# nomadkaraoke/python-audio-separator

Hardware: AMD Instinct MI355X
Metric: audio-sec separated / wall-sec (RTF), UVR-MDX-NET 44.1kHz stereo, 1/2/4/8 GPU (higher is better)
Workload: dtype f32 (I/O and accumulators; matrix products on the 16-bit pipe from block-scaled two-part fp16 operands, 22-bit products -- see arithmetic; fp32-exact setting timed in arithmetic_ab)

## Files before the change

python-audio-separator_amd/csrc/asx.hip:

```cpp
#include <hip/hip_runtime.h>

#include <algorithm>
#include <atomic>
#include <cmath>
#include <cstdarg>
#include <cstdio>
#include <cstdlib>
#include <cstring>
#include <functional>
#include <map>
#include <string>
#include <mutex>
#include <vector>

#include "../../include/asx.h"
#include "knobs.h"
#include "resample_plan.h"
#include "flac_dec_plan.h"

static void grant_lds(const void *kernel, int bytes) {
  static std::mutex mu;
  static std::map<const void *, int> granted;
  std::lock_guard<std::mutex> lock(mu);
  int &g = granted[kernel];
// ... 29 lines not shown
#include "kernels_pcm_encode.h"
#include "kernels_flac_dec.h"

using namespace asx;

#include "engine_core.h"
#include "engine_mdx.h"

static int opt_nonneg(int32_t v) { return v < 0 ? 0 : (int)v; }
static int opt_onoff(int32_t v) { return v > 0 ? 1 : 0; }

static const struct EngineOption {
  const char *key;
  int asx_engine::*field;
  int EngineKnobs::*knob;
  int (*norm)(int32_t);
  const char *refusal = nullptr;
  int shipped = 0;
} kOptions[] = {
    {"winograd", &asx_engine::winograd, &EngineKnobs::winograd, opt_nonneg,
     "asx_set_option: winograd = %d names a superseded kernel generation that only an experimental build carries "
     "(python build.py --experimental); this library has 0 (direct kernel) and 3 (the default)", 3},
    {"winograd_stationary", &asx_engine::winos, &EngineKnobs::winos, opt_nonneg,
     "asx_set_option: the weight-stationary Winograd kernel (measured slower) is in experimental builds only (python build.py --experimental)"},
    {"winograd_bf16x6", &asx_engine::wino6, &EngineKnobs::wino6, opt_nonneg},
    {"gemm_bf16x6", &asx_engine::gemm_bf16x6, &EngineKnobs::gemm_bf16x6, opt_onoff},
    {"gemm_f16x3", &asx_engine::gemm_f16x3, &EngineKnobs::gemm_f16x3, opt_onoff},
    {"conv_direct_f16x3", &asx_engine::conv3h, &EngineKnobs::conv3h, opt_nonneg},
    {"conv_fuse_input", &asx_engine::conv_fuse_input, &EngineKnobs::conv_fuse_input, opt_onoff},
    {"tdf_fuse_output", &asx_engine::tdf_fuse_output, &EngineKnobs::tdf_fuse_output, opt_onoff},
    {"conv3h_partial_scratch", &asx_engine::conv3h_ps, &EngineKnobs::conv3h_ps, opt_onoff},
    {"conv3h_walk", &asx_engine::conv3h_walk, &EngineKnobs::conv3h_walk, opt_onoff},
    {"conv3h_tiled", &asx_engine::conv3h_tiled, &EngineKnobs::conv3h_tiled, opt_onoff},
    {"conv_down_bf16x6", &asx_engine::down6, &EngineKnobs::down6, opt_onoff},
    {"conv_up_bf16x6", &asx_engine::up6, &EngineKnobs::up6, opt_onoff},
    {"gemm_pair_images", &asx_engine::pair_images, &EngineKnobs::pair_images, opt_onoff,
     "asx_set_option: gemm_pair_images = 1 needs an experimental build (python build.py --experimental): the pair-image reader measured no "
     "faster in the nets and is not in the default library"},
};

static const EngineOption *find_option(const char *fn, const char *key) {
  for (const EngineOption &o : kOptions)
    if (!strcmp(key, o.key)) return &o;
  set_err("%s: unknown option '%s'", fn, key);
  return nullptr;
}

extern "C" {

int asx_abi_version(void) { return ASX_ABI_VERSION; }
const char *asx_last_error(void) { return g_err; }

int asx_device_count(void) {
  int n = 0;
  if (hipGetDeviceCount(&n) != hipSuccess) return 0;
  return n;
}

int asx_engine_create(int device, const asx_mdx_config *cfg, asx_engine **out) {
  REQUIRE(cfg && out, "asx_engine_create: null argument");
  REQUIRE(cfg->n_fft >= 8 && cfg->n_fft % 2 == 0, "n_fft must be even and >= 8 (got %d)", cfg->n_fft);
  REQUIRE(cfg->hop_length > 0 && cfg->segment_size >= 2, "bad hop_length/segment_size");
  REQUIRE(cfg->dim_f > 0 && cfg->dim_f <= cfg->n_fft / 2 + 1, "dim_f %d out of range for n_fft %d", cfg->dim_f,
          cfg->n_fft);
  REQUIRE(cfg->overlap >= 0.0 && cfg->overlap < 1.0, "overlap must be in [0,1)");
  REQUIRE(cfg->win_length >= 0 && cfg->win_length <= cfg->n_fft, "win_length %d out of range for n_fft %d", cfg->win_length, cfg->n_fft);
// ... 2600 lines not shown

int asx_vr_separate(asx_engine *e, const float *wave_host, int64_t n_samples, const asx_vr_params *params, float *primary_host,
                    float *secondary_host) {
  REQUIRE(e && wave_host && params && n_samples > 0, "asx_vr_separate: bad argument");
  READY(e->vr, "asx_vr_separate");
  HIPCHK(hipSetDevice(e->device));
  int T;
  int64_t n_out;
  CHK(vr_plan(*e->vr, n_samples, &T, &n_out));
  DevBuf dw, dp, ds;
  BufGuard g{{&dw, &dp, &ds}};
  CHK(to_dev(dw, wave_host, (size_t)2 * n_samples));
  if (primary_host) CHK(dp.ensure((size_t)2 * n_out * 4));
  if (secondary_host) CHK(ds.ensure((size_t)2 * n_out * 4));
  CHK(vr_separate_dev(e, dw.f(), n_samples, params, primary_host ? dp.f() : nullptr, secondary_host ? ds.f() : nullptr, nullptr));
  if (primary_host) CHK(to_host(primary_host, dp, (size_t)2 * n_out));
  if (secondary_host) CHK(to_host(secondary_host, ds, (size_t)2 * n_out));
  return ASX_OK;
}

int asx_counter(const asx_engine *e, const char *name, int64_t *out) {
  REQUIRE(e && name && out, "asx_counter: null argument");
  const std::string nm(name);
  if (nm == "tdf3_launches") *out = (int64_t)g_tdf3_launches.load();
  else if (nm == "tdf3h_launches") *out = (int64_t)g_tdf3h_launches.load();
  else if (nm == "attn6_launches") *out = (int64_t)g_attn6_launches.load();
  else if (nm == "attn6h_launches") *out = (int64_t)g_attn6h_launches.load();
  else if (nm == "tdf3_gather_launches") *out = (int64_t)g_tdf3_gather_launches.load();
  else if (nm == "wino6_launches") *out = (int64_t)g_wino6_launches.load();
  else if (nm == "wino6h_launches") *out = (int64_t)g_wino6h_launches.load();
  else if (nm == "conv3h_launches") *out = (int64_t)g_conv3h_launches.load();
  else if (nm == "conv3h_fin_launches") *out = (int64_t)g_conv3h_fin_launches.load();
  else if (nm == "conv3h_tiled_launches") *out = (int64_t)g_conv3h_tiled_launches.load();
  else if (nm == "tdf_fused_output_launches") *out = (int64_t)g_tdf_fused_output_launches.load();
  else if (nm == "tdf3_pair_image_launches") *out = (int64_t)g_tdf3ps_launches.load();
  else if (nm == "down6_launches") *out = (int64_t)g_down6_launches.load();
  else if (nm == "up6_launches") *out = (int64_t)g_up6_launches.load();
  else if (nm == "hd_rounds") *out = (int64_t)g_hd_rounds.load();
  else if (nm == "vr_net_passes") *out = (int64_t)g_vr_net_passes.load();
  else if (nm == "v3_net_passes") *out = (int64_t)g_v3_net_passes.load();
  else if (nm == "rof_net_passes") *out = (int64_t)g_rof_net_passes.load();
  else if (nm == "flac_block_cycles") *out = (int64_t)e->flac_block_cycles;
  else if (nm == "flac_crc16_cycles") *out = (int64_t)e->flac_crc16_cycles;
  else {
    set_err("asx_counter: unknown counter '%s'", name);
    return ASX_ERR_INVALID;
  }
  return ASX_OK;
}

int asx_debug_trace(uint64_t *host, int64_t n_u64) {
  REQUIRE(host && n_u64 > 0 && n_u64 <= 4096 * 8, "asx_debug_trace: bad argument");
  HIPCHK(hipDeviceSynchronize());
  HIPCHK(hipMemcpyFromSymbol(host, HIP_SYMBOL(asx_dbg_trace), (size_t)n_u64 * 8));
  return ASX_OK;
}

int asx_debug_fetch(asx_engine *e, const char *name, float *host, int64_t numel) {
  REQUIRE(e && name && host && numel > 0, "asx_debug_fetch: bad argument");
  HIPCHK(hipSetDevice(e->device));
  const float *src = nullptr;
  const std::string nm(name);
  if (e->vr && e->vr->ws_batch > 0) {
    auto &b = e->vr->b;
    if (nm == "vr.hc") src = b.hc;
    else if (nm == "vr.y2") src = b.y2;
// ... 249 lines not shown
```

python-audio-separator_amd/csrc/conv3h_walk_plan.h:

```cpp
#pragma once
#include <algorithm>
#include <cstdint>
#include <vector>

struct Conv3hUnit {
  int32_t b, band, t0, tiles;
};

struct Conv3hWalkPlan {
  int bw = 32, tps = 0;
  int ngroups = 8;
  std::vector<std::vector<Conv3hUnit>> units;
  int steps(int g) const {
    int n = 0;
    for (const Conv3hUnit &u : units[(size_t)g]) n += u.tiles + 1;
    return n;
  }
  int longest() const {
    int n = 0;
    for (int g = 0; g < ngroups; ++g) n = std::max(n, steps(g));
    return n;
  }
  int max_units() const {
    size_t n = 0;
    for (const auto &l : units) n = std::max(n, l.size());
    return (int)n;
  }
};

static inline int conv3h_walk_bw0(int B, int tilesT, int tilesF) {
  int bw = 32;
  double best = 1e30;
  for (int cand : {32, 16, 8}) {
    if ((tilesT * cand) % 32 != 0) continue;
    const int tps = tilesT * cand / 32;
    const int bands = (tilesF + cand - 1) / cand, items = B * bands;
    const double cost = (double)(bands * cand) / tilesF * (tps + 1.0) / tps * (double)((items + 7) / 8) / (items / 8.0);
    if (cost < best - 1e-9) {
      best = cost;
      bw = cand;
    }
  }
  return best > 1e29 ? 32 : bw;
}

static inline Conv3hWalkPlan conv3h_walk_arith(int B, int tilesT, int tilesF, int bw) {
  Conv3hWalkPlan p;
  p.bw = (tilesT * bw) % 32 == 0 ? bw : 32;
  p.tps = tilesT * p.bw / 32;
  const int segs = 32 / p.bw, nbands = (tilesF + p.bw - 1) / p.bw, items = B * nbands;
  p.ngroups = 8 * segs;
  p.units.assign((size_t)p.ngroups, {});
  for (int x = 0; x < 8; ++x)
    for (int seg = 0; seg < segs; ++seg)
      for (int item = x; item < items; item += 8)
        p.units[(size_t)(x * segs + seg)].push_back({item / nbands, item % nbands, seg * p.tps, p.tps});
  return p;
}
static inline Conv3hWalkPlan conv3h_walk_plan0(int B, int tilesT, int tilesF) { return conv3h_walk_arith(B, tilesT, tilesF, conv3h_walk_bw0(B, tilesT, tilesF)); }

static inline Conv3hWalkPlan conv3h_walk_balanced(int B, int tilesT, int tilesF, int gran, int bw) {
  Conv3hWalkPlan p;
  p.bw = bw;
  p.tps = 0;
  p.ngroups = 256 / bw;
  p.units.assign((size_t)p.ngroups, {});
  const int G = p.ngroups, nbands = (tilesF + bw - 1) / bw, items = B * nbands;
  const int rounds = items / G, left = items - rounds * G;
  for (int r = 0; r < rounds; ++r)
    for (int g = 0; g < G; ++g) {
      const int item = r * G + g;
      p.units[(size_t)g].push_back({item / nbands, item % nbands, 0, tilesT});
    }
  if (left > 0) {
    const int64_t tT = ((int64_t)(tilesT + gran - 1) / gran) * gran, total = (int64_t)left * tT;
    int64_t share = (total + G - 1) / G;
    share = (share + gran - 1) / gran * gran;
    for (int g = 0; g < G; ++g) {
      int64_t lo = (int64_t)g * share;
      const int64_t hi = std::min(total, lo + share);
      while (lo < hi) {
        const int64_t i = lo / tT, t0 = lo - i * tT, t1 = std::min<int64_t>(tT, t0 + (hi - lo));
        const int item = rounds * G + (int)i;
        if (t0 < tilesT) p.units[(size_t)g].push_back({item / nbands, item % nbands, (int)t0, (int)std::min<int64_t>(t1, tilesT) - (int)t0});
        lo += t1 - t0;
      }
    }
  }
  return p;
}

static inline Conv3hWalkPlan conv3h_walk_plan(int B, int tilesT, int tilesF, int gran, int mode) {
  Conv3hWalkPlan best = conv3h_walk_plan0(B, tilesT, tilesF);
  if (mode == 0) return best;
  if (gran < 1) gran = 1;
  int nbest = best.tps % gran == 0 || best.tps == tilesT ? best.longest() : INT32_MAX;
  for (int bw : {32, 16, 8}) {
    Conv3hWalkPlan c = conv3h_walk_balanced(B, tilesT, tilesF, gran, bw);
    const int n = c.longest();
    if (n < nbest) {
      nbest = n;
      best = std::move(c);
    }
  }
  return best;
}

static inline int conv3h_walk_table(const Conv3hWalkPlan &p, std::vector<int32_t> &tab) {
  const int stride = p.max_units() + 2;
  tab.assign((size_t)p.ngroups * stride * 4, 0);
  for (int g = 0; g < p.ngroups; ++g) {
    int32_t *row = &tab[(size_t)g * stride * 4];
    const auto &l = p.units[(size_t)g];
    row[0] = p.steps(g);
    row[1] = (int32_t)l.size();
    for (size_t u = 0; u <= l.size(); ++u) {
      const Conv3hUnit un = u < l.size() ? l[u] : Conv3hUnit{0, 0, 0, 1 << 30};
      int32_t *e = row + 4 * (1 + u);
      e[0] = un.b;
      e[1] = un.band;
      e[2] = un.t0;
      e[3] = un.tiles;
    }
  }
  return stride;
// ... 2 lines not shown
```

python-audio-separator_amd/csrc/engine_core.h:

```cpp
#pragma once

static thread_local char g_err[512] = "";
static void set_err(const char *fmt, ...) {
  va_list ap;
  va_start(ap, fmt);
  vsnprintf(g_err, sizeof(g_err), fmt, ap);
  va_end(ap);
}
#define HIPCHK(x)                                                                       \
  do {                                                                                  \
    hipError_t e_ = (x);                                                                \
    if (e_ != hipSuccess) {                                                             \
      set_err("%s:%d %s -> %s", __FILE__, __LINE__, #x, hipGetErrorString(e_));         \
      return ASX_ERR_HIP;                                                               \
    }                                                                                   \
  } while (0)
#define CHK(x)                    \
  do {                            \
    int r_ = (x);                 \
    if (r_ != ASX_OK) return r_;  \
  } while (0)
#define REQUIRE(cond, ...)        \
  do {                            \
    if (!(cond)) {                \
// ... 80 lines not shown
  DevBuf wd6;
  int wd6_cg = 0, wd6_nst = 0, wd6_nrep = 3;
  DevBuf wup6;
  int wup6_cg = 0, wup6_nst = 0;
};

struct TdfLayer {
  int n = 0, k = 0, c = 0;
  bool has_bias = false;
  DevBuf w, bias, scale, shift;
  DevBuf gn_w, gn_b;
};

struct Block {
  std::vector<ConvLayer> tfc;
  TdfLayer tdf0, tdf1;
  int c = 0, t = 0, f = 0;
};

struct ProfRec {
  int cls;
  int nprod;
  hipEvent_t a, b;
  double flops, bytes;
};

struct RsTable {
  ResamplePlan plan;
  DevBuf tab;
};

struct Conv3hWalkTab {
  int B, tilesT, tilesF, mode;
  int bw, stride;
  DevBuf tab;
};

struct V3Net;
struct RofNet;
struct HtNet;
struct HdNet;
struct VrNet;
struct EnsCtx;

struct W3Entry {
  const float *w;
  int N, K, cin;
  int kind;
  void *img;
};

struct DivKey {
  int64_t N = -1;
  int n_chunks = 0;
  int64_t C = 0, step = 0, L = 0;
  int trim = 0, win = 0;
  int hann_tab = 0;
  bool operator==(const DivKey &o) const {
    return N == o.N && n_chunks == o.n_chunks && C == o.C && step == o.step && L == o.L && trim == o.trim && win == o.win &&
           hann_tab == o.hann_tab;
  }
};

struct asx_engine {
  int device = 0;
  V3Net *v3 = nullptr;
// ... 25 lines not shown
  std::vector<ConvLayer> ds, us;
  int ws_batch = 0;
  DevBuf spec_in, spec_out, R[3], H, HE, frames, chunk_out, d_starts, d_nact, d_peak, d_demixed;
  DevBuf pool_wave, pool_nsong, pool_songs, pool_div, pool_peak;
  DevBuf c3h_ps;
  std::vector<Conv3hWalkTab *> c3h_walks;
  DevBuf gn_part;
  DevBuf d_div;
  DivKey div_key;
  DevBuf sinc_tab;
  DevBuf sinc_jobs;
  DevBuf flac_cycles;
  long long flac_block_cycles = 0, flac_crc16_cycles = 0;
  DevBuf flac_frames, flac_off;
  DevBuf flacdec_list, flacdec_slots, flacdec_accept;
  std::vector<flacdec::Accept> flacdec_accept_host;
  int64_t flacdec_n_samples = -1, flacdec_n_frames = 0;
  int32_t flacdec_channels = 0, flacdec_bps = 0, flacdec_max_bs = 0;
  size_t flacdec_slot_off = 0;
  std::vector<RsTable *> rs_tabs;
  std::mutex rs_mu;
  hipEvent_t div_ev = nullptr;
  hipStream_t div_stream = nullptr;
  std::vector<DevBuf> skip;
  int winograd = 3;
  int winos = 0;
  int gemm_bf16x6 = 1;
  int gemm_f16x3 = 1;
  int wino6 = 144;
  int conv3h = 144;
  int conv3h_ps = 1;
  int conv3h_walk = 1;
  int conv3h_tiled = 1;
  int conv_fuse_input = 1;
  int tdf_fuse_output = 1;
  int down6 = 1;
  int up6 = 1;
  int pair_images = 0;
  std::vector<W3Entry> w3;
  std::mutex w3_mu;
  bool prof = false;
  int prof_nprod = 0;
  std::vector<ProfRec> recs;
};

static int pick_batch(const asx_engine *e) { return e->cfg.max_batch > 0 ? e->cfg.max_batch : 64; }

#include "batching.h"

template <class F>
static int timed(asx_engine *e, int cls, double flops, double bytes, hipStream_t s, F &&launch) {
  if (!e->prof) {
    launch();
    HIPCHK(hipGetLastError());
    return ASX_OK;
  }
  ProfRec r;
  r.cls = cls;
  r.flops = flops;
  r.bytes = bytes;
  HIPCHK(hipEventCreate(&r.a));
  HIPCHK(hipEventCreate(&r.b));
  HIPCHK(hipEventRecord(r.a, s));
  e->prof_nprod = 0;
  launch();
  r.nprod = e->prof_nprod;
// ... 57 lines not shown
```

python-audio-separator_amd/csrc/engine_mdx.h:

```cpp
#pragma once

template <class CFG>
static void launch_conv_t(const ConvArgs &a, int nblk, hipStream_t s) {
  grant_lds(&conv_mfma_kernel<CFG>, CFG::LDS_BYTES);
  hipLaunchKernelGGL(conv_mfma_kernel<CFG>, dim3(nblk), dim3(256), CFG::LDS_BYTES, s, a);
}

static int conv_tile_h(int kind) { return kind == CK_UP ? 4 : 8; }

static int pick_nrep_conv(int cout) {
  const int ct = (cout + 15) / 16;
  int best = 1, best_pad = 1 << 30;
  for (int n = 3; n >= 1; --n) {
    const int pad = ((ct + n - 1) / n) * n - ct;
    if (pad < best_pad) {
      best_pad = pad;
      best = n;
    }
  }
  return best;
}
static int pick_nrep_up(int cout) {
  const int ct = (cout + 15) / 16;
  if (knobs().up_nrep == 4 && (4 * ct) % 4 == 0) return 4;
// ... 170 lines not shown
    else down6_pack<3>(w, L.cout, L.cin, w6, &L.wd6_cg, &L.wd6_nst);
    CHK(L.wd6.ensure(w6.size() * 4));
    HIPCHK(hipMemcpy(L.wd6.p, w6.data(), w6.size() * 4, hipMemcpyHostToDevice));
  }
  if (L.kind == CK_UP) {
    std::vector<uint32_t> w6;
    if (L.nrep == 6) up6_pack<6>(w, L.cout, L.cin, w6, &L.wup6_cg, &L.wup6_nst);
    else if (L.nrep == 4) up6_pack<4>(w, L.cout, L.cin, w6, &L.wup6_cg, &L.wup6_nst);
    else up6_pack<2>(w, L.cout, L.cin, w6, &L.wup6_cg, &L.wup6_nst);
    CHK(L.wup6.ensure(w6.size() * 4));
    HIPCHK(hipMemcpy(L.wup6.p, w6.data(), w6.size() * 4, hipMemcpyHostToDevice));
  }
  const int nb = (L.kind == CK_UP) ? CT * 16 : std::max(L.cg * NW, ((L.cout + 47) / 48) * 48);
  std::vector<float> bp(nb, 0.f);
  for (int i = 0; i < L.cout; ++i) bp[i] = b ? b[i] : 0.f;
  CHK(L.w.ensure(wp.size() * 4));
  CHK(L.b.ensure(bp.size() * 4));
  HIPCHK(hipMemcpy(L.w.p, wp.data(), wp.size() * 4, hipMemcpyHostToDevice));
  HIPCHK(hipMemcpy(L.b.p, bp.data(), bp.size() * 4, hipMemcpyHostToDevice));
  return ASX_OK;
}

template <class CFG>
static void launch_conv_dma_t(const ConvArgs &a, int nblk, hipStream_t s) {
  grant_lds(&conv_dma_kernel<CFG>, CFG::LDS_BYTES);
  hipLaunchKernelGGL(conv_dma_kernel<CFG>, dim3(nblk), dim3(256), CFG::LDS_BYTES, s, a);
}

static std::atomic<long long> g_wino6_launches{0};
static std::atomic<long long> g_wino6h_launches{0};
static std::atomic<long long> g_conv3h_launches{0};
static std::atomic<long long> g_conv3h_fin_launches{0};
static std::atomic<long long> g_conv3h_tiled_launches{0};
static std::atomic<long long> g_down6_launches{0};
static std::atomic<long long> g_up6_launches{0};

struct ConvView {
  int64_t x_bstride = 0;
  int64_t y_bstride = 0;
  const float *res = nullptr;
  int64_t aux_bstride = 0;
  int act = -1;
  float alpha = 1.f;
  const ConvLayer *fin = nullptr;
  const float *fin_x = nullptr;
  bool x_tiled = false, y_tiled = false;
};

static bool conv3h_takes(const asx_engine *e, const ConvLayer &L, bool dma, const float *res, int act, int T, int F, int64_t y_bstride, const float *y) {
#ifdef ASX_EXPERIMENTAL_KERNELS
  if (e->winos == 1 && L.wus.p != nullptr) return false;
#endif
  return L.kind == CK_3X3 && e->winograd == 3 && e->gemm_bf16x6 > 0 && e->gemm_f16x3 > 0 && e->conv3h > 0 && L.cin <= e->conv3h && L.w3h.p != nullptr && dma &&
         res == nullptr && (act == ACT_RELU || act == ACT_NONE) && F % 32 == 0 && (int64_t)Conv3hCfg::C * T * F < ((int64_t)1 << 29) &&
         y_bstride % 4 == 0 && (reinterpret_cast<uintptr_t>(y) & 15) == 0;
}

static bool conv3h_tiled_ok(const asx_engine *e, const ConvLayer &L, int T) { return T % 4 == 0 && (L.cin == Conv3hCfg::C || e->conv3h_ps > 0); }

static size_t conv3h_ps_need(const ConvLayer &L, int B, int T, int F) {
  if (L.kind != CK_3X3 || L.w3h.p == nullptr || L.cin <= Conv3hCfg::C || F % 32 != 0 || B <= 0 || T <= 0) return 0;
  return (size_t)Conv3hCfg::ps_bytes(B, (T + 3) / 4, F / 32);
}

static const Conv3hWalkTab *conv3h_walk_find(const asx_engine *e, int B, int tilesT, int tilesF, int mode) {
  for (const Conv3hWalkTab *t : e->c3h_walks)
    if (t->B == B && t->tilesT == tilesT && t->tilesF == tilesF && t->mode == mode) return t;
  return nullptr;
}
static int conv3h_walk_ensure(asx_engine *e, const ConvLayer &L, int B, int T, int F) {
  if (L.kind != CK_3X3 || L.w3h.p == nullptr || F % 32 != 0 || B <= 0 || T <= 0) return ASX_OK;
  const int tilesT = (T + 3) / 4, tilesF = F / 32;
  for (int mode = 0; mode < 2; ++mode) {
    if (conv3h_walk_find(e, B, tilesT, tilesF, mode)) continue;
    const Conv3hWalkPlan plan = conv3h_walk_plan(B, tilesT, tilesF, 1, mode);
    std::vector<int32_t> tab;
    Conv3hWalkTab *t = new Conv3hWalkTab{B, tilesT, tilesF, mode, plan.bw, conv3h_walk_table(plan, tab), DevBuf()};
    int rc = t->tab.ensure(tab.size() * 4);
    if (rc == ASX_OK && hipMemcpy(t->tab.p, tab.data(), tab.size() * 4, hipMemcpyHostToDevice) != hipSuccess) {
      set_err("conv3h_walk_ensure: the upload of a walk table failed");
      rc = ASX_ERR_HIP;
    }
    if (rc != ASX_OK) {
      t->tab.release();
      delete t;
      return rc;
    }
    e->c3h_walks.push_back(t);
  }
  return ASX_OK;
}

static int conv_launch(asx_engine *e, const ConvLayer &L, const float *x, const float *skip, float *y, int B, int T,
                       int F, hipStream_t s, const ConvView &v = ConvView()) {
  ConvArgs a{};
  a.x = x;
  a.wp = L.w.f();
  a.bias = L.b.f();
  a.skip = skip;
  a.res = v.res;
  a.zeros = e->d_zeros.f();
  a.y = y;
  a.B = B;
  a.Cin = L.cin;
  a.Cout = L.cout;
  a.T = T;
  a.F = F;
  a.act = v.act >= 0 ? v.act : (L.relu ? ACT_RELU : ACT_NONE);
  a.alpha = v.alpha;
  REQUIRE(a.act != ACT_ELU || L.kind == CK_1X1, "ELU epilogue: 1x1 convolutions only");
// ... 51 lines not shown
    wa.tilesF = a.Fo / 32;
    const int NS = (a.To + 1) / 2;
    const int base = wa.CG * wa.tilesF * B;
    int RB = std::max(1, std::min((NS + 7) / 8, (2048 + base - 1) / base));
    const int SPB = (NS + RB - 1) / RB;
    RB = (NS + SPB - 1) / SPB;
    wa.tilesT = RB;
    wa.NCI = SPB;
    const int nb = base * RB;
    auto gos = [&](auto kern, int lds) {
      grant_lds(kern, lds);
      return timed(e, cls, flops, bytes, s, [&]() { hipLaunchKernelGGL(kern, dim3(nb), dim3(512), lds, s, wa); });
    };
    const int abls = knobs().winos_abl;
    const bool k12 = L.wus_ks == 12;
    const bool ragged = (a.To & 1) || (L.cout % 48) != 0;
    if (abls && !ragged) {
      switch (abls) {
        case 1: return k12 ? gos(&conv_winos_kernel<12, 1>, WinoSCfg<12>::LDS_BYTES) : gos(&conv_winos_kernel<24, 1>, WinoSCfg<24>::LDS_BYTES);
        case 2: return k12 ? gos(&conv_winos_kernel<12, 2>, WinoSCfg<12>::LDS_BYTES) : gos(&conv_winos_kernel<24, 2>, WinoSCfg<24>::LDS_BYTES);
        case 4: return k12 ? gos(&conv_winos_kernel<12, 4>, WinoSCfg<12>::LDS_BYTES) : gos(&conv_winos_kernel<24, 4>, WinoSCfg<24>::LDS_BYTES);
        case 5: return k12 ? gos(&conv_winos_kernel<12, 5>, WinoSCfg<12>::LDS_BYTES) : gos(&conv_winos_kernel<24, 5>, WinoSCfg<24>::LDS_BYTES);
        case 13: return k12 ? gos(&conv_winos_kernel<12, 13>, WinoSCfg<12>::LDS_BYTES) : gos(&conv_winos_kernel<24, 13>, WinoSCfg<24>::LDS_BYTES);
        default: break;
      }
    }
    if (ragged) return k12 ? gos(&conv_winos_kernel<12, 0, true>, WinoSCfg<12>::LDS_BYTES) : gos(&conv_winos_kernel<24, 0, true>, WinoSCfg<24>::LDS_BYTES);
    return k12 ? gos(&conv_winos_kernel<12, 0, false>, WinoSCfg<12>::LDS_BYTES) : gos(&conv_winos_kernel<24, 0, false>, WinoSCfg<24>::LDS_BYTES);
  }
#endif
  if (conv3h_takes(e, L, dma, v.res, a.act, T, F, a.y_bstride, y)) {
    const int nb = L.cin / Conv3hCfg::C;
    const int tilesT = (T + 3) / 4, tilesF = F / 32;
    const Conv3hWalkTab *wt = conv3h_walk_find(e, B, tilesT, tilesF, e->conv3h_walk > 0 ? 1 : 0);
    REQUIRE(wt != nullptr, "conv3h_kernel: no walk table for %d x %d x %d (the workspace set-up plans them)", B, T, F);
    grant_lds(&conv3h_kernel<0, false>, Conv3hCfg::LDS_BYTES);
    grant_lds(&conv3h_kernel<0, true>, Conv3hCfg::LDS_BYTES);
    grant_lds(&conv3h_kernel<0, false, true>, Conv3hCfg::LDS_BYTES);
    grant_lds(&conv3h_kernel<0, false, false, 1>, Conv3hCfg::LDS_BYTES);
    grant_lds(&conv3h_kernel<0, false, false, 2>, Conv3hCfg::LDS_BYTES);
    grant_lds(&conv3h_kernel<0, false, false, 3>, Conv3hCfg::LDS_BYTES);
    auto go = [&](auto finc, auto psc, const Conv3hArgs &ca, bool yt) {
      constexpr bool FIN = decltype(finc)::value;
      constexpr int PS = decltype(psc)::value;
      auto one = [&](auto kern) {
        grant_lds(kern, Conv3hCfg::LDS_BYTES);
        hipLaunchKernelGGL(kern, dim3(256), dim3(512), Conv3hCfg::LDS_BYTES, s, ca);
      };
      if constexpr (FIN) {
        if (yt) one(&conv3h_kernel<0, false, true, 0, false, true>);
        else one(&conv3h_kernel<0, false, true>);
      } else if constexpr ((PS & 2) != 0) {
        if (v.x_tiled) one(&conv3h_kernel<0, false, false, PS, true, false>);
        else one(&conv3h_kernel<0, false, false, PS>);
      } else {
        if (v.x_tiled && yt) one(&conv3h_kernel<0, false, false, PS, true, true>);
        else if (v.x_tiled) one(&conv3h_kernel<0, false, false, PS, true, false>);
        else if (yt) one(&conv3h_kernel<0, false, false, PS, false, true>);
        else one(&conv3h_kernel<0, false, false, PS>);
      }
      if (v.x_tiled || yt) g_conv3h_tiled_launches.fetch_add(1);
    };
    const int64_t plane = (int64_t)T * F;
    const bool ps = e->conv3h_ps > 0 && nb > 1;
    const int64_t ps_item = Conv3hCfg::ps_item_bytes(tilesT, tilesF);
    REQUIRE(!ps || (ps_item < ((int64_t)1 << 32) && e->c3h_ps.p != nullptr && e->c3h_ps.bytes >= conv3h_ps_need(L, B, T, F)),
            "conv3h_kernel: the partial-sum scratch is not sized for %d x %d x %d (the workspace set-up sizes it)", B, T, F);
    Conv3hArgs walk{};
    walk.B = B;
    walk.T = T;
    walk.F = F;
    walk.x_bstride = a.x_bstride;
    walk.y_bstride = a.y_bstride;
    walk.tilesT = tilesT;
    walk.tilesF = tilesF;
    walk.bw = wt->bw;
    walk.walk = reinterpret_cast<const u32x4 *>(wt->tab.p);
    walk.walk_stride = wt->stride;
    walk.ps = ps ? e->c3h_ps.p : nullptr;
    walk.ps_bstride = ps_item;
    return timed(e, cls, flops, bytes, s, [&]() {
      e->prof_nprod = 3;
      for (int ob = 0; ob < nb; ++ob)
        for (int ib = 0; ib < nb; ++ib) {
          Conv3hArgs ca = walk;
          ca.x = x + (int64_t)ib * Conv3hCfg::C * plane;
          ca.y = y + (int64_t)ob * Conv3hCfg::C * plane;
          ca.prev = ib > 0 && !ps ? ca.y : nullptr;
          ca.wimg = reinterpret_cast<const u32x4 *>(reinterpret_cast<const uint32_t *>(L.w3h.p) + (size_t)(ob * nb + ib) * Conv3hCfg::IMG_U32);
          ca.bias = ib == 0 ? L.b.f() + ob * Conv3hCfg::C : nullptr;
          ca.act = ib == nb - 1 ? a.act : ACT_NONE;
          if (v.fin) {
            ca.xin = v.fin_x;
            ca.xin_bstride = 4 * plane;
            ca.w1 = v.fin->w1f.f();
            go(std::true_type{}, IntC<0>{}, ca, v.y_tiled);
            g_conv3h_fin_launches.fetch_add(1);
          } else if (ps && ib == 0) go(std::false_type{}, IntC<2>{}, ca, false);
          else if (ps && ib < nb - 1) go(std::false_type{}, IntC<3>{}, ca, false);
          else if (ps) go(std::false_type{}, IntC<1>{}, ca, v.y_tiled);
          else if (ib > 0) hipLaunchKernelGGL((conv3h_kernel<0, true>), dim3(256), dim3(512), Conv3hCfg::LDS_BYTES, s, ca);
          else go(std::false_type{}, IntC<0>{}, ca, v.y_tiled);
          g_conv3h_launches.fetch_add(1);
        }
    });
  }
  if (L.kind == CK_3X3 && e->winograd == 3 && e->gemm_bf16x6 > 0 && e->wino6 > 0 && L.cin >= e->wino6 && dma && L.wu6_nci > 0 &&
      (int64_t)T * F < ((int64_t)1 << 24)) {
    ConvArgs wa = a;
    const bool h3 = e->gemm_f16x3 > 0 && L.wu6h.p != nullptr;
    wa.wp = reinterpret_cast<const float *>(h3 ? L.wu6h.p : L.wu6.p);
    wa.CG = L.wu_cg;
    wa.NCI = L.wu6_nci;
// ... 900 lines not shown
```

python-audio-separator_amd/csrc/kernels_conv3h.h:

```cpp
#pragma once
#include <cstring>
#include <vector>

#include "conv3h_walk_plan.h"
#include "kernels_gemm3.h"

namespace asx {

struct Conv3hArgs {
  const float *x;
  float *y;
  const u32x4 *wimg;
  const float *bias;
  int B, T, F;
  int64_t x_bstride, y_bstride;
  int act;
  int tilesT, tilesF;
  int bw;
  const u32x4 *walk;
  int walk_stride;
  const float *prev;
  long long *dbg;
  const float *xin;
  const float *w1;
  int64_t xin_bstride;
  void *ps;
  int64_t ps_bstride;
};

struct Conv3hCfg {
  static constexpr int C = 48, CG8 = C / 8;
  static constexpr int TH = 4, TW = 32, IW = TW + 2;
  static constexpr int PSTR = C * 2;
  static constexpr int ROWB = IW * PSTR;
  static constexpr int RING = 12;
  static constexpr int PART = RING * ROWB;
  static constexpr int KGY = 3 * CG8;
  static constexpr int SPK = (KGY + 3) / 4;
  static constexpr int NST = (3 * KGY + 3) / 4;
  static constexpr int WKY = (KGY / 4) * 3 * 2 * 1024 + 3 * 2 * 512;
  static constexpr int WBYTES = 3 * WKY;
  static constexpr int W_OFF = 0, X_OFF = WBYTES, TAB_OFF = X_OFF + 2 * PART;
  static constexpr int LDS_BYTES = TAB_OFF + 64;
  static constexpr size_t IMG_U32 = WBYTES / 4 + 48;
  static constexpr int EUP = 8;
  static constexpr int EQ = 8;

  static constexpr int PS_STORE = 1024, PS_WAVE = 6 * PS_STORE, PS_TILE = 4 * PS_WAVE;
  static constexpr int64_t ps_item_bytes(int tilesT, int tilesF) { return (int64_t)tilesF * tilesT * PS_TILE; }
  static constexpr int64_t ps_bytes(int B, int tilesT, int tilesF) { return (int64_t)B * ps_item_bytes(tilesT, tilesF); }
  static constexpr unsigned ps_wave_off(int tilesT, int strip, int jt, int r) { return (unsigned)((strip * tilesT + jt) * 4 + r) * (unsigned)PS_WAVE; }
  static constexpr int64_t ps_off(int tilesT, int tilesF, int b, int strip, int jt, int r, int k, int lane) {
    return (int64_t)b * ps_item_bytes(tilesT, tilesF) + ps_wave_off(tilesT, strip, jt, r) + k * PS_STORE + lane * 16;
  }

  static constexpr int TL_BLOCK = 1024, TL_PIECE = 16;
  static constexpr int64_t tl_item_bytes(int T, int F) { return (int64_t)C * T * F * 4; }
  static constexpr unsigned tl_block_off(int F, int t, int ftile, int n) { return ((unsigned)(t * (F / 16) + ftile) * 3u + (unsigned)n) * (unsigned)TL_BLOCK; }
  static constexpr unsigned tl_in_block(int g, int ch) { return (unsigned)(g * 256 + ch * TL_PIECE); }
  static constexpr int64_t tl_off(int T, int F, int t, int f, int c) {
// ... 112 lines not shown
      const int nl = half ? 32 : 64;
      for (int n = 0; n < 3; ++n)
        for (int lane = 0; lane < nl; ++lane) {
          const int co = n * 16 + (lane & 15);
          const int kk = 4 * sg + (lane >> 4);
          const int tap = ky * 3 + kk / CFG::CG8, c0 = (kk % CFG::CG8) * 8;
          uint16_t hh[8], ll[8];
          for (int e = 0; e < 8; ++e) {
            const float us = ldexpf(w[((size_t)co * C + c0 + e) * 9 + tap], ex[co]);
            hh[e] = conv3h_f16_rne(us);
            ll[e] = conv3h_f16_rne(us - conv3h_f16_f(hh[e]));
          }
          const size_t pstep = half ? 512 : 1024;
          const size_t fb = (size_t)ky * CFG::WKY + (half ? (size_t)(CFG::SPK - 1) * 6144 + (size_t)(n * 2) * 512 : (size_t)sg * 6144 + (size_t)(n * 2) * 1024);
          uint32_t *dh = &img[(fb + (size_t)lane * 16) / 4], *dl = &img[(fb + pstep + (size_t)lane * 16) / 4];
          for (int e = 0; e < 4; ++e) {
            dh[e] = (uint32_t)hh[2 * e] | ((uint32_t)hh[2 * e + 1] << 16);
            dl[e] = (uint32_t)ll[2 * e] | ((uint32_t)ll[2 * e + 1] << 16);
          }
        }
    }
}

struct Conv3hWalk {
  int u, j, b, strip, t0, tiles;
};
__device__ __forceinline__ void conv3h_walk_unit(const Conv3hArgs &a, int wg, Conv3hWalk &w) {
  const u32x4 un = a.walk[w.u];
  w.b = __builtin_amdgcn_readfirstlane((int)un.x);
  w.strip = __builtin_amdgcn_readfirstlane((int)un.y) * a.bw + ((wg >> 3) & (a.bw - 1));
  w.t0 = __builtin_amdgcn_readfirstlane((int)un.z);
  w.tiles = __builtin_amdgcn_readfirstlane((int)un.w);
}
__device__ __forceinline__ int conv3h_walk_row(const Conv3hArgs &a, int wg) {
  const int sh = __builtin_ctz((unsigned)a.bw);
  return ((wg & 7) * (32 >> sh) + ((wg >> 3) >> sh)) * a.walk_stride;
}
__device__ __forceinline__ int conv3h_row0(const Conv3hWalk &w) { return w.t0 * 4; }
__device__ __forceinline__ int conv3h_nblocks(const Conv3hArgs &a, int wg) { return (int)a.walk[conv3h_walk_row(a, wg)].x; }
__device__ __forceinline__ void conv3h_walk_init(const Conv3hArgs &a, int wg, Conv3hWalk &w) {
  w.u = conv3h_walk_row(a, wg) + 1;
  w.j = -1;
  conv3h_walk_unit(a, wg, w);
}
__device__ __forceinline__ void conv3h_walk_next(const Conv3hArgs &a, int wg, Conv3hWalk &w) {
  if (++w.j == w.tiles) {
    w.j = -1;
    ++w.u;
    conv3h_walk_unit(a, wg, w);
  }
}

__device__ __forceinline__ void conv3h_split_pair(float x0, float x1, float s, unsigned &h, unsigned &l) {
  unsigned hh = 0, ll = 0;
  asm("v_fma_mixlo_f16 %0, %1, %2, 0 op_sel_hi:[0,0,0]" : "+v"(hh) : "v"(x0), "v"(s));
  asm("v_fma_mixhi_f16 %0, %1, %2, 0 op_sel_hi:[0,0,0]" : "+v"(hh) : "v"(x1), "v"(s));
  asm("v_fma_mixlo_f16 %0, %1, %2, -%3 op_sel:[0,0,0] op_sel_hi:[0,0,1]" : "+v"(ll) : "v"(x0), "v"(s), "v"(hh));
  asm("v_fma_mixhi_f16 %0, %1, %2, -%3 op_sel:[0,0,1] op_sel_hi:[0,0,1]" : "+v"(ll) : "v"(x1), "v"(s), "v"(hh));
  h = hh;
  l = ll;
}

template <int BM>
__device__ __forceinline__ float ror8m(float keep, float from) {
  return __builtin_bit_cast(float, __builtin_amdgcn_update_dpp(__builtin_bit_cast(int, keep), __builtin_bit_cast(int, from), 0x128, 0xf, BM, false));
}

template <bool FIN>
struct Conv3hFinRegs {};
template <>
struct Conv3hFinRegs<true> {
  f32x4 rin[4][4];
  bool ok[4];
  float w1[8][4], b1[8];
};

template <int ABL = 0, bool ACC = false, bool FIN = false, int PS = 0, bool XT = false, bool YT = false>
__global__ __launch_bounds__(512) __attribute__((amdgpu_waves_per_eu(2, 2))) void conv3h_kernel(Conv3hArgs a) {
  using CFG = Conv3hCfg;
  constexpr bool PIN = (PS & 1) != 0, POUT = (PS & 2) != 0;
  constexpr bool OWNQ = POUT || YT;
  static_assert(!(PS != 0 && (ACC || FIN)), "partial sums through the scratch: neither the planar accumulate mode nor the fused input");
  static_assert(!(XT && (FIN || ACC)) && !(YT && (ACC || POUT)), "tile order: never the accumulate mode; the fused input has no input slice, a partial-out launch no final output");
  extern __shared__ float lds_f[];
  char *lds = reinterpret_cast<char *>(lds_f);
  const int tid = threadIdx.x;
  const int lane = tid & 63;
  const int wave = __builtin_amdgcn_readfirstlane(tid >> 6);
  const int wg = blockIdx.x;
  float *maxtab = reinterpret_cast<float *>(lds + CFG::TAB_OFF);
  int *exps = reinterpret_cast<int *>(lds + CFG::TAB_OFF + 32);

  {
    const u32x4 *src = a.wimg;
    u32x4 *dst = reinterpret_cast<u32x4 *>(lds + CFG::W_OFF);
    for (int i = tid; i < CFG::WBYTES / 16; i += 512) dst[i] = src[i];
  }
  const int64_t TF = (int64_t)a.T * a.F;
  const int NB = __builtin_amdgcn_readfirstlane(conv3h_nblocks(a, wg));
  const unsigned plane_bytes = (unsigned)(CFG::C * TF * 4);

  if (wave >= 4) {
    const int ptid = tid - 256, pw = wave - 4;
    int row, cig, q;
    if (ptid < 160) {
      q = (ptid & 1) + 2 * ((ptid >> 3) % 5);
      cig = (ptid >> 1) & 3;
      row = ptid / 40;
    } else {
      const int u = ptid - 160;
      q = (u & 1) + 2 * ((u >> 3) % 5);
      cig = 4 + ((u >> 1) & 1);
      row = ((u >> 2) & 1) + 2 * (u / 40);
    }
    const bool item_ok = ptid < 240;
    const int loff = (row * CFG::IW + 4 * q - 3) * CFG::PSTR + cig * 16;
    const int goff = FIN ? (int)((int64_t)row * a.F + 4 * q)
                         : (int)(((int64_t)cig * 8 * a.T + row) * a.F + 4 * q);
    const unsigned tl_lane = CFG::tl_fetch_lane(a.F, row, cig, q);
    constexpr int NSET = FIN ? 2 : 4;
    f32x4 raw[NSET][8];
    Conv3hFinRegs<FIN> fr;
    const unsigned in_bytes = (unsigned)(4 * TF * 4);
    if constexpr (FIN) {
#pragma unroll
      for (int c = 0; c < 8; ++c) {
        const f32x4 wv = *reinterpret_cast<const f32x4 *>(a.w1 + (cig * 8 + c) * 4);
        fr.w1[c][0] = wv.x;
        fr.w1[c][1] = wv.y;
        fr.w1[c][2] = wv.z;
        fr.w1[c][3] = wv.w;
        fr.b1[c] = a.w1[CFG::C * 4 + cig * 8 + c];
      }
    }

    Conv3hWalk wk;
    conv3h_walk_init(a, wg, wk);
    int nf = 0;
    auto fetch = [&](auto setc) {
      constexpr int S = decltype(setc)::value;
      const int tb = nf < NB ? wk.b : 0, f0 = wk.strip * 32;
      const int t1 = nf < NB ? conv3h_row0(wk) + wk.j * 4 + 1 : -(1 << 20);
      ++nf;
      conv3h_walk_next(a, wg, wk);
      __amdgpu_buffer_rsrc_t rs = FIN ? __builtin_amdgcn_make_buffer_rsrc(const_cast<float *>(a.xin + (int64_t)tb * a.xin_bstride), 0, in_bytes, 0x00020000)
                                      : __builtin_amdgcn_make_buffer_rsrc(const_cast<float *>(a.x + (int64_t)tb * a.x_bstride), 0, plane_bytes, 0x00020000);
      const int org = t1 * a.F + (f0 - 4);
      const bool ok = item_ok && (unsigned)(t1 + row) < (unsigned)a.T && (unsigned)(f0 - 4 + 4 * q) < (unsigned)a.F;
      const unsigned vo = !ok ? 0xfffffff0u
                              : (XT ? tl_lane + CFG::tl_fetch_org(a.F, t1, f0) : (unsigned)(goff + org) * 4u);
      if constexpr (FIN) {
        fr.ok[S] = ok;
#pragma unroll
        for (int j = 0; j < 4; ++j) fr.rin[S][j] = __builtin_bit_cast(f32x4, __builtin_amdgcn_raw_buffer_load_b128(rs, (int)vo, (int)(j * TF * 4), 0));
      } else {
#pragma unroll
        for (int j = 0; j < 8; ++j) {
          if constexpr ((ABL & 2) != 0) raw[S][j] = (f32x4){0.25f, 0.5f, 0.75f, 1.f};
          else raw[S][j] = __builtin_bit_cast(f32x4, __builtin_amdgcn_raw_buffer_load_b128(rs, (int)vo, XT ? j * CFG::TL_PIECE : (int)(j * TF * 4), 0));
        }
      }
    };
    auto tile_max = [&](auto setc, int slot) {
      constexpr int S = decltype(setc)::value % NSET;
      if constexpr (FIN) {
        constexpr int SI = decltype(setc)::value;
        const bool ok = fr.ok[SI];
        auto px = [&](float i0, float i1, float i2, float i3, int c) {
          const float v = __builtin_fmaf(fr.w1[c][3], i3, __builtin_fmaf(fr.w1[c][2], i2, __builtin_fmaf(fr.w1[c][1], i1, __builtin_fmaf(fr.w1[c][0], i0, fr.b1[c]))));
          return ok ? __builtin_fmaxf(v, 0.f) : 0.f;
// ... 168 lines not shown
#pragma unroll
      for (int qq = 0; qq < 2; ++qq) {
        v[qq].x = __builtin_fmaf(pacc[qq][c].x, sc, bz[c]);
        v[qq].y = __builtin_fmaf(pacc[qq][c].y, sc, bz[c]);
        v[qq].z = __builtin_fmaf(pacc[qq][c].z, sc, bz[c]);
        v[qq].w = __builtin_fmaf(pacc[qq][c].w, sc, bz[c]);
        if constexpr (PIN) v[qq] += pprev[c * 2 + qq];
      }
      f32x4 o;
      if constexpr (K % 2 == 0) o = (f32x4){ror8m<0xC>(v[0].x, v[1].x), ror8m<0xC>(v[0].y, v[1].y), ror8m<0xC>(v[0].z, v[1].z), ror8m<0xC>(v[0].w, v[1].w)};
      else o = (f32x4){ror8m<0x3>(v[1].x, v[0].x), ror8m<0x3>(v[1].y, v[0].y), ror8m<0x3>(v[1].z, v[0].z), ror8m<0x3>(v[1].w, v[0].w)};
      if constexpr (ACC) o += pprev[K];
      pend[K] = (f32x4){fmaxf(o.x, act_lo), fmaxf(o.y, act_lo), fmaxf(o.z, act_lo), fmaxf(o.w, act_lo)};
    };
    auto flush = [&]() {
      epi_chunk(IntC<0>{});
      epi_chunk(IntC<1>{});
      epi_chunk(IntC<2>{});
      epi_chunk(IntC<3>{});
      epi_chunk(IntC<4>{});
      epi_chunk(IntC<5>{});
      flush_one(IntC<0>{});
      flush_one(IntC<1>{});
      flush_one(IntC<2>{});
      flush_one(IntC<3>{});
      flush_one(IntC<4>{});
      flush_one(IntC<5>{});
      pend_rs = __builtin_amdgcn_make_buffer_rsrc(a.y, 0, 0, 0x00020000);
    };

    __syncthreads();
    __syncthreads();
    Conv3hWalk wk;
    conv3h_walk_init(a, wg, wk);
    int s3 = 0;
    for (int s = 0; s < NB; ++s) {
      const int tb = wk.b, j = wk.j, wk_strip = wk.strip, wk_t0 = wk.t0, f0 = wk_strip * 32;
      conv3h_walk_next(a, wg, wk);
      if constexpr ((ABL & 32) != 0) {
        if (wg == 0 && wave == 0 && s < 64) {
          const long long t = __builtin_amdgcn_s_memtime();
          if (lane == 0) a.dbg[s * 8 + 4] = t;
        }
      }
      if (j >= 0) {
        const int tt = (wk_t0 + j) * 4 + wave;
        const bool cur_ok = tt < a.T && f0 < a.F;
        const int cur_vo = (((li & 7) * a.T + tt) * a.F + f0 + ((li >> 3) * 4 + g) * 4) * 4;
        const int cur_ps = (int)CFG::ps_wave_off(a.tilesT, wk_strip, wk_t0 + j, wave);
        const int cur_tl = (int)CFG::tl_store_off(a.F, tt, f0, 0);
        const int sp = s3 == 0 ? 2 : s3 - 1;
        const int e_cur = __builtin_amdgcn_readfirstlane(exps[s3]), e_old = __builtin_amdgcn_readfirstlane(exps[sp]);
        int rowoff[3], eky[3];
#pragma unroll
        for (int ky = 0; ky < 3; ++ky) {
          const int u = wave + ky;
          rowoff[ky] = (u < 2 ? sp * 4 + 2 + u : s3 * 4 + u - 2) * CFG::ROWB;
          eky[ky] = u < 2 ? e_old : e_cur;
        }
        const int xm = (pad_lane ? rowoff[MST.kyb] : rowoff[MST.ky]) + vl[CFG::SPK - 1];
        f32x4 acc[2][3];
#pragma unroll
        for (int p = 0; p < 2; ++p)
#pragma unroll
          for (int c = 0; c < 3; ++c) acc[p][c] = (f32x4){0.f, 0.f, 0.f, 0.f};
        constexpr int PF = (ABL & 2048) ? 2 : 1;
        f16x8 wf[PF + 1][3][2], xf[PF + 1][2][2];
// ... 131 lines not shown
```

python-audio-separator_amd/csrc/knobs.h:

```cpp
#pragma once

#include <algorithm>
#include <climits>
#include <cstdint>
#include <cstdlib>

#ifndef ASX_TDF2_DEFAULT
#define ASX_TDF2_DEFAULT 1
#endif

constexpr int HD_MAX_GROUPS = 6;

namespace knob {
inline bool set(const char *name) { return getenv(name) != nullptr; }
inline int num(const char *name, int def) { return set(name) ? atoi(getenv(name)) : def; }
inline int64_t num64(const char *name, int64_t def) { return set(name) ? atoll(getenv(name)) : def; }
inline double real(const char *name, double def) { return set(name) ? atof(getenv(name)) : def; }
inline bool on_unless_0(const char *name) { return !(set(name) && atoi(getenv(name)) == 0); }
inline bool off_unless_nonzero(const char *name) { return set(name) && atoi(getenv(name)) != 0; }
inline int clamped(const char *name, int def, int lo, int hi = INT_MAX) { return set(name) ? std::max(lo, std::min(hi, atoi(getenv(name)))) : def; }
}

struct Knobs {
  int poison = knob::num("ASX_POISON", -1);
// ... 52 lines not shown
  int attn_qw = knob::num("ASX_ATTN_QW", 1);
  bool attn6 = knob::on_unless_0("ASX_ATTN6");
  int attn6_qw = knob::num("ASX_ATTN6_QW", 2);
  bool attn_v1 = knob::off_unless_nonzero("ASX_ATTN_V1");
  bool rof_normfuse = knob::on_unless_0("ASX_ROF_NORMFUSE");
  int rof_gelu = knob::num("ASX_ROF_GELU", 2);
  bool rof_fuse = knob::on_unless_0("ASX_ROF_FUSE");
};

inline const Knobs &knobs() {
  static const Knobs k;
  return k;
}

struct EngineKnobs {
#ifdef ASX_EXPERIMENTAL_KERNELS
  int winograd = knob::clamped("ASX_WINOGRAD", 3, 0);
  int winos = knob::clamped("ASX_WINOS", 0, 0);
  int pair_images = knob::num("ASX_PAIR_IMAGES", 0);
#else
  int winograd = knob::num("ASX_WINOGRAD", 3) <= 0 ? 0 : 3;
  int winos = 0;
  int pair_images = 0;
#endif
  int gemm_bf16x6 = knob::num("ASX_GEMM_BF16X6", 1);
  int gemm_f16x3 = knob::num("ASX_GEMM_F16X3", 1);
  int wino6 = knob::clamped("ASX_WINO6", 144, 0);
  int conv3h = knob::clamped("ASX_CONV3H", 144, 0);
  int conv_fuse_input = 1;
  int tdf_fuse_output = 1;
  int conv3h_ps = 1;
  int conv3h_walk = 1;
  int conv3h_tiled = 1;
  int down6 = knob::num("ASX_DOWN6", 1);
  int up6 = knob::num("ASX_UP6", 1);
  bool fft3 = knob::on_unless_0("ASX_FFT3");
  bool fft3p = knob::on_unless_0("ASX_FFT3P");
};
```

Baseline: 1725.

## Merge per-output-block conv3h launches into one dispatch over all output blocks

New measurement: 1750, median of 6. 1.01x the previous value.

```diff
diff --git a/python-audio-separator_amd/csrc/asx.hip b/python-audio-separator_amd/csrc/asx.hip
--- a/python-audio-separator_amd/csrc/asx.hip
+++ b/python-audio-separator_amd/csrc/asx.hip
@@ -85,6 +85,7 @@
     {"conv3h_partial_scratch", &asx_engine::conv3h_ps, &EngineKnobs::conv3h_ps, opt_onoff},
     {"conv3h_walk", &asx_engine::conv3h_walk, &EngineKnobs::conv3h_walk, opt_onoff},
     {"conv3h_tiled", &asx_engine::conv3h_tiled, &EngineKnobs::conv3h_tiled, opt_onoff},
+    {"conv3h_merge_out", &asx_engine::conv3h_merge, &EngineKnobs::conv3h_merge, opt_nonneg},
     {"conv_down_bf16x6", &asx_engine::down6, &EngineKnobs::down6, opt_onoff},
     {"conv_up_bf16x6", &asx_engine::up6, &EngineKnobs::up6, opt_onoff},
     {"gemm_pair_images", &asx_engine::pair_images, &EngineKnobs::pair_images, opt_onoff,
@@ -2751,6 +2752,7 @@
   else if (nm == "conv3h_launches") *out = (int64_t)g_conv3h_launches.load();
   else if (nm == "conv3h_fin_launches") *out = (int64_t)g_conv3h_fin_launches.load();
   else if (nm == "conv3h_tiled_launches") *out = (int64_t)g_conv3h_tiled_launches.load();
+  else if (nm == "conv3h_merged_dispatches") *out = (int64_t)g_conv3h_merged_dispatches.load();
   else if (nm == "tdf_fused_output_launches") *out = (int64_t)g_tdf_fused_output_launches.load();
   else if (nm == "tdf3_pair_image_launches") *out = (int64_t)g_tdf3ps_launches.load();
   else if (nm == "down6_launches") *out = (int64_t)g_down6_launches.load();
diff --git a/python-audio-separator_amd/csrc/conv3h_walk_plan.h b/python-audio-separator_amd/csrc/conv3h_walk_plan.h
--- a/python-audio-separator_amd/csrc/conv3h_walk_plan.h
+++ b/python-audio-separator_amd/csrc/conv3h_walk_plan.h
@@ -10,6 +10,7 @@
 struct Conv3hWalkPlan {
   int bw = 32, tps = 0;
   int ngroups = 8;
+  int nob = 1;
   std::vector<std::vector<Conv3hUnit>> units;
   int steps(int g) const {
     int n = 0;
@@ -59,11 +60,31 @@
 }
 static inline Conv3hWalkPlan conv3h_walk_plan0(int B, int tilesT, int tilesF) { return conv3h_walk_arith(B, tilesT, tilesF, conv3h_walk_bw0(B, tilesT, tilesF)); }
 
-static inline Conv3hWalkPlan conv3h_walk_balanced(int B, int tilesT, int tilesF, int gran, int bw) {
+#if defined(__HIPCC__)
+#define CONV3H_WALK_HD __host__ __device__
+#else
+#define CONV3H_WALK_HD
+#endif
+CONV3H_WALK_HD static inline void conv3h_walk_wg(int wg, int bw, int nob, int &row, int &ob) {
+  const int gx = 32 / bw, x = wg & 7, seg = (wg >> 3) / bw;
+  if (nob < 1) nob = 1;
+  if (gx % nob == 0) {
+    row = x * (gx / nob) + seg / nob;
+    ob = seg % nob;
+  } else {
+    const int g = x * gx + seg;
+    row = g / nob;
+    ob = g % nob;
+    if (row >= (8 * gx) / nob) row = -1;
+  }
+}
+
+static inline Conv3hWalkPlan conv3h_walk_balanced(int B, int tilesT, int tilesF, int gran, int bw, int nob = 1) {
   Conv3hWalkPlan p;
   p.bw = bw;
   p.tps = 0;
-  p.ngroups = 256 / bw;
+  p.nob = nob;
+  p.ngroups = (256 / bw) / nob;
   p.units.assign((size_t)p.ngroups, {});
   const int G = p.ngroups, nbands = (tilesF + bw - 1) / bw, items = B * nbands;
   const int rounds = items / G, left = items - rounds * G;
@@ -90,7 +111,33 @@
   return p;
 }
 
-static inline Conv3hWalkPlan conv3h_walk_plan(int B, int tilesT, int tilesF, int gran, int mode) {
+static inline Conv3hWalkPlan conv3h_walk_dealt(int B, int tilesT, int tilesF, int bw, int nob) {
+  Conv3hWalkPlan p;
+  p.bw = bw;
+  p.tps = tilesT;
+  p.nob = nob;
+  p.ngroups = (256 / bw) / nob;
+  p.units.assign((size_t)p.ngroups, {});
+  const int nbands = (tilesF + bw - 1) / bw, items = B * nbands;
+  for (int item = 0; item < items; ++item) p.units[(size_t)(item % p.ngroups)].push_back({item / nbands, item % nbands, 0, tilesT});
+  return p;
+}
+
+static inline Conv3hWalkPlan conv3h_walk_plan(int B, int tilesT, int tilesF, int gran, int mode, int nob = 1) {
+  if (nob > 1) {
+    if (gran < 1) gran = 1;
+    Conv3hWalkPlan best;
+    int nbest = INT32_MAX;
+    for (int bw : {32, 16, 8}) {
+      Conv3hWalkPlan c = mode == 0 ? conv3h_walk_dealt(B, tilesT, tilesF, bw, nob) : conv3h_walk_balanced(B, tilesT, tilesF, gran, bw, nob);
+      const int n = c.longest();
+      if (n <= nbest) {
+        nbest = n;
+        best = std::move(c);
+      }
+    }
+    return best;
+  }
   Conv3hWalkPlan best = conv3h_walk_plan0(B, tilesT, tilesF);
   if (mode == 0) return best;
   if (gran < 1) gran = 1;
diff --git a/python-audio-separator_amd/csrc/engine_core.h b/python-audio-separator_amd/csrc/engine_core.h
--- a/python-audio-separator_amd/csrc/engine_core.h
+++ b/python-audio-separator_amd/csrc/engine_core.h
@@ -136,6 +136,7 @@
 
 struct Conv3hWalkTab {
   int B, tilesT, tilesF, mode;
+  int nob;
   int bw, stride;
   DevBuf tab;
 };
@@ -227,6 +228,7 @@
   int conv3h_ps = 1;
   int conv3h_walk = 1;
   int conv3h_tiled = 1;
+  int conv3h_merge = 144;
   int conv_fuse_input = 1;
   int tdf_fuse_output = 1;
   int down6 = 1;
diff --git a/python-audio-separator_amd/csrc/engine_mdx.h b/python-audio-separator_amd/csrc/engine_mdx.h
--- a/python-audio-separator_amd/csrc/engine_mdx.h
+++ b/python-audio-separator_amd/csrc/engine_mdx.h
@@ -226,6 +226,7 @@
 static std::atomic<long long> g_conv3h_launches{0};
 static std::atomic<long long> g_conv3h_fin_launches{0};
 static std::atomic<long long> g_conv3h_tiled_launches{0};
+static std::atomic<long long> g_conv3h_merged_dispatches{0};
 static std::atomic<long long> g_down6_launches{0};
 static std::atomic<long long> g_up6_launches{0};
 
@@ -254,22 +255,23 @@
 
 static size_t conv3h_ps_need(const ConvLayer &L, int B, int T, int F) {
   if (L.kind != CK_3X3 || L.w3h.p == nullptr || L.cin <= Conv3hCfg::C || F % 32 != 0 || B <= 0 || T <= 0) return 0;
-  return (size_t)Conv3hCfg::ps_bytes(B, (T + 3) / 4, F / 32);
-}
-
-static const Conv3hWalkTab *conv3h_walk_find(const asx_engine *e, int B, int tilesT, int tilesF, int mode) {
+  return (size_t)(L.cin / Conv3hCfg::C) * (size_t)Conv3hCfg::ps_bytes(B, (T + 3) / 4, F / 32);
+}
+
+static const Conv3hWalkTab *conv3h_walk_find(const asx_engine *e, int B, int tilesT, int tilesF, int mode, int nob) {
   for (const Conv3hWalkTab *t : e->c3h_walks)
-    if (t->B == B && t->tilesT == tilesT && t->tilesF == tilesF && t->mode == mode) return t;
+    if (t->B == B && t->tilesT == tilesT && t->tilesF == tilesF && t->mode == mode && t->nob == nob) return t;
   return nullptr;
 }
 static int conv3h_walk_ensure(asx_engine *e, const ConvLayer &L, int B, int T, int F) {
   if (L.kind != CK_3X3 || L.w3h.p == nullptr || F % 32 != 0 || B <= 0 || T <= 0) return ASX_OK;
-  const int tilesT = (T + 3) / 4, tilesF = F / 32;
-  for (int mode = 0; mode < 2; ++mode) {
-    if (conv3h_walk_find(e, B, tilesT, tilesF, mode)) continue;
-    const Conv3hWalkPlan plan = conv3h_walk_plan(B, tilesT, tilesF, 1, mode);
+  const int tilesT = (T + 3) / 4, tilesF = F / 32, nb = L.cin / Conv3hCfg::C;
+  for (int k = 0; k < (nb > 1 ? 4 : 2); ++k) {
+    const int mode = k & 1, nob = k < 2 ? 1 : nb;
+    if (conv3h_walk_find(e, B, tilesT, tilesF, mode, nob)) continue;
+    const Conv3hWalkPlan plan = conv3h_walk_plan(B, tilesT, tilesF, 1, mode, nob);
     std::vector<int32_t> tab;
-    Conv3hWalkTab *t = new Conv3hWalkTab{B, tilesT, tilesF, mode, plan.bw, conv3h_walk_table(plan, tab), DevBuf()};
+    Conv3hWalkTab *t = new Conv3hWalkTab{B, tilesT, tilesF, mode, nob, plan.bw, conv3h_walk_table(plan, tab), DevBuf()};
     int rc = t->tab.ensure(tab.size() * 4);
     if (rc == ASX_OK && hipMemcpy(t->tab.p, tab.data(), tab.size() * 4, hipMemcpyHostToDevice) != hipSuccess) {
       set_err("conv3h_walk_ensure: the upload of a walk table failed");
@@ -387,7 +389,9 @@
   if (conv3h_takes(e, L, dma, v.res, a.act, T, F, a.y_bstride, y)) {
     const int nb = L.cin / Conv3hCfg::C;
     const int tilesT = (T + 3) / 4, tilesF = F / 32;
-    const Conv3hWalkTab *wt = conv3h_walk_find(e, B, tilesT, tilesF, e->conv3h_walk > 0 ? 1 : 0);
+    const bool ps = e->conv3h_ps > 0 && nb > 1;
+    const bool merged = ps && L.cin <= e->conv3h_merge;
+    const Conv3hWalkTab *wt = conv3h_walk_find(e, B, tilesT, tilesF, e->conv3h_walk > 0 ? 1 : 0, merged ? nb : 1);
     REQUIRE(wt != nullptr, "conv3h_kernel: no walk table for %d x %d x %d (the workspace set-up plans them)", B, T, F);
     grant_lds(&conv3h_kernel<0, false>, Conv3hCfg::LDS_BYTES);
     grant_lds(&conv3h_kernel<0, true>, Conv3hCfg::LDS_BYTES);
@@ -414,10 +418,9 @@
         else if (yt) one(&conv3h_kernel<0, false, false, PS, false, true>);
         else one(&conv3h_kernel<0, false, false, PS>);
       }
-      if (v.x_tiled || yt) g_conv3h_tiled_launches.fetch_add(1);
+      if (v.x_tiled || yt) g_conv3h_tiled_launches.fetch_add(ca.nob);
     };
     const int64_t plane = (int64_t)T * F;
-    const bool ps = e->conv3h_ps > 0 && nb > 1;
     const int64_t ps_item = Conv3hCfg::ps_item_bytes(tilesT, tilesF);
     REQUIRE(!ps || (ps_item < ((int64_t)1 << 32) && e->c3h_ps.p != nullptr && e->c3h_ps.bytes >= conv3h_ps_need(L, B, T, F)),
             "conv3h_kernel: the partial-sum scratch is not sized for %d x %d x %d (the workspace set-up sizes it)", B, T, F);
@@ -434,6 +437,29 @@
     walk.walk_stride = wt->stride;
     walk.ps = ps ? e->c3h_ps.p : nullptr;
     walk.ps_bstride = ps_item;
+    walk.nob = 1;
+    if (merged)
+      return timed(e, cls, flops, bytes, s, [&]() {
+        e->prof_nprod = 3;
+        for (int ib = 0; ib < nb; ++ib) {
+          Conv3hArgs ca = walk;
+          ca.nob = nb;
+          ca.x = x + (int64_t)ib * Conv3hCfg::C * plane;
+          ca.y = y;
+          ca.y_ostride = (int64_t)Conv3hCfg::C * plane;
+          ca.wimg = reinterpret_cast<const u32x4 *>(reinterpret_cast<const uint32_t *>(L.w3h.p) + (size_t)ib * Conv3hCfg::IMG_U32);
+          ca.wimg_ostride = (int64_t)nb * (Conv3hCfg::IMG_U32 / 4);
+          ca.bias = ib == 0 ? L.b.f() : nullptr;
+          ca.bias_ostride = Conv3hCfg::C;
+          ca.ps_ostride = Conv3hCfg::ps_bytes(B, tilesT, tilesF);
+          ca.act = ib == nb - 1 ? a.act : ACT_NONE;
+          if (ib == 0) go(std::false_type{}, IntC<2>{}, ca, false);
+          else if (ib < nb - 1) go(std::false_type{}, IntC<3>{}, ca, false);
+          else go(std::false_type{}, IntC<1>{}, ca, v.y_tiled);
+          g_conv3h_launches.fetch_add(nb);
+          g_conv3h_merged_dispatches.fetch_add(1);
+        }
+      });
     return timed(e, cls, flops, bytes, s, [&]() {
       e->prof_nprod = 3;
       for (int ob = 0; ob < nb; ++ob)
diff --git a/python-audio-separator_amd/csrc/kernels_conv3h.h b/python-audio-separator_amd/csrc/kernels_conv3h.h
--- a/python-audio-separator_amd/csrc/kernels_conv3h.h
+++ b/python-audio-separator_amd/csrc/kernels_conv3h.h
@@ -26,6 +26,9 @@
   int64_t xin_bstride;
   void *ps;
   int64_t ps_bstride;
+  int nob;
+  int64_t wimg_ostride, bias_ostride, y_ostride;
+  int64_t ps_ostride;
 };
 
 struct Conv3hCfg {
@@ -204,14 +207,22 @@
   w.t0 = __builtin_amdgcn_readfirstlane((int)un.z);
   w.tiles = __builtin_amdgcn_readfirstlane((int)un.w);
 }
+template <bool MO>
 __device__ __forceinline__ int conv3h_walk_row(const Conv3hArgs &a, int wg) {
+  if constexpr (MO) {
+    int row, ob;
+    conv3h_walk_wg(wg, a.bw, a.nob, row, ob);
+    return row * a.walk_stride;
+  }
   const int sh = __builtin_ctz((unsigned)a.bw);
   return ((wg & 7) * (32 >> sh) + ((wg >> 3) >> sh)) * a.walk_stride;
 }
 __device__ __forceinline__ int conv3h_row0(const Conv3hWalk &w) { return w.t0 * 4; }
-__device__ __forceinline__ int conv3h_nblocks(const Conv3hArgs &a, int wg) { return (int)a.walk[conv3h_walk_row(a, wg)].x; }
+template <bool MO>
+__device__ __forceinline__ int conv3h_nblocks(const Conv3hArgs &a, int wg) { return (int)a.walk[conv3h_walk_row<MO>(a, wg)].x; }
+template <bool MO>
 __device__ __forceinline__ void conv3h_walk_init(const Conv3hArgs &a, int wg, Conv3hWalk &w) {
-  w.u = conv3h_walk_row(a, wg) + 1;
+  w.u = conv3h_walk_row<MO>(a, wg) + 1;
   w.j = -1;
   conv3h_walk_unit(a, wg, w);
 }
@@ -252,6 +263,7 @@
   using CFG = Conv3hCfg;
   constexpr bool PIN = (PS & 1) != 0, POUT = (PS & 2) != 0;
   constexpr bool OWNQ = POUT || YT;
+  constexpr bool MO = PS != 0;
   static_assert(!(PS != 0 && (ACC || FIN)), "partial sums through the scratch: neither the planar accumulate mode nor the fused input");
   static_assert(!(XT && (FIN || ACC)) && !(YT && (ACC || POUT)), "tile order: never the accumulate mode; the fused input has no input slice, a partial-out launch no final output");
   extern __shared__ float lds_f[];
@@ -262,6 +274,15 @@
   const int wg = blockIdx.x;
   float *maxtab = reinterpret_cast<float *>(lds + CFG::TAB_OFF);
   int *exps = reinterpret_cast<int *>(lds + CFG::TAB_OFF + 32);
+  if constexpr (MO) {
+    int row, ob;
+    conv3h_walk_wg(wg, a.bw, a.nob, row, ob);
+    if (row < 0) return;
+    a.wimg += ob * a.wimg_ostride;
+    if (a.bias) a.bias += ob * a.bias_ostride;
+    a.y += ob * a.y_ostride;
+    a.ps = static_cast<char *>(a.ps) + ob * a.ps_ostride;
+  }
 
   {
     const u32x4 *src = a.wimg;
@@ -269,7 +290,7 @@
     for (int i = tid; i < CFG::WBYTES / 16; i += 512) dst[i] = src[i];
   }
   const int64_t TF = (int64_t)a.T * a.F;
-  const int NB = __builtin_amdgcn_readfirstlane(conv3h_nblocks(a, wg));
+  const int NB = __builtin_amdgcn_readfirstlane(conv3h_nblocks<MO>(a, wg));
   const unsigned plane_bytes = (unsigned)(CFG::C * TF * 4);
 
   if (wave >= 4) {
@@ -307,7 +328,7 @@
     }
 
     Conv3hWalk wk;
-    conv3h_walk_init(a, wg, wk);
+    conv3h_walk_init<MO>(a, wg, wk);
     int nf = 0;
     auto fetch = [&](auto setc) {
       constexpr int S = decltype(setc)::value;
@@ -542,7 +563,7 @@
     __syncthreads();
     __syncthreads();
     Conv3hWalk wk;
-    conv3h_walk_init(a, wg, wk);
+    conv3h_walk_init<MO>(a, wg, wk);
     int s3 = 0;
     for (int s = 0; s < NB; ++s) {
       const int tb = wk.b, j = wk.j, wk_strip = wk.strip, wk_t0 = wk.t0, f0 = wk_strip * 32;
diff --git a/python-audio-separator_amd/csrc/knobs.h b/python-audio-separator_amd/csrc/knobs.h
--- a/python-audio-separator_amd/csrc/knobs.h
+++ b/python-audio-separator_amd/csrc/knobs.h
@@ -108,6 +108,7 @@
   int conv3h_ps = 1;
   int conv3h_walk = 1;
   int conv3h_tiled = 1;
+  int conv3h_merge = 144;
   int down6 = knob::num("ASX_DOWN6", 1);
   int up6 = knob::num("ASX_UP6", 1);
   bool fft3 = knob::on_unless_0("ASX_FFT3");
```
